# jafarinia/snuffy

Measured on AMD Instinct MI355X. Metric: slides/sec, higher is better.
Workload: dtype f32; 1 GPU; cfgB: MILNet eval forward, 1 bag/step/rank, N=32768 patches D=768 h=6 Lambda=200 (K=200) depth=1 relu mlp x4; parallelism=bag-parallel x1, bags_resident_per_rank=8, launch=hip graph replay, rccl_ranks=0

## Files before the change

### snuffy_amd/csrc/gemm.hip

```cpp
#include <stdlib.h>

#include "mfma.h"
#include "philox.h"

namespace {

struct GemmParams {
    const unsigned short* a;
    const unsigned short* w;
    const float* bias;
    void* c;
    int64_t lda, ldw, ldc;
    int m, n, k;
    int act;
    int tiles_m, tiles_n;
    unsigned long long* trace;
    const float* resid = nullptr;
    int64_t ldr = 0;
    unsigned int* split_cnt = nullptr;
    float* split_slab = nullptr;
    int split_cap = 0, split_rcap = 0;
    const unsigned short* gate = nullptr;
    int64_t ldg = 0;
    const float* colsum = nullptr;
// ... 402 lines not shown
    while (true) {
        const int next = tile + wgs_per_xcd;
        const bool has_next = next < t_hi;
        const Src nxt = tile_src(has_next ? next : tile);
        const bool full = (tile / P.tiles_n + 1) * BM <= P.m && (tile % P.tiles_n + 1) * BN <= P.n;
        for (int s = 0; s < ns; ++s) {
            if constexpr (EPI == 2)
                if (s == 0) preload_x(tile);
            read_frags(rb);
            if (s == ns - 1) load_bias(tile);
            const bool in_tile = s + AHEAD < ns;
            const int exist = has_next ? AHEAD : (ns - 1 - s < AHEAD ? ns - 1 - s : AHEAD);
            if (in_tile)
                stage(cur, s + AHEAD, sb);
            else if (has_next)
                stage(nxt, s + AHEAD - ns, sb);
            if (exist == AHEAD) {
                if (after_epilogue)
                    wait_vmcnt<(AHEAD - 1) * GL + MI * NST>();
                else
                    wait_vmcnt<(AHEAD - 1) * GL>();
            } else if (AHEAD == 3 && exist == 2) {
                wait_vmcnt<GL>();
            } else {
                wait_vmcnt<0>();
            }
            after_epilogue = false;
            rb = rb == NBUF - 1 ? 0 : rb + 1;
            sb = sb == NBUF - 1 ? 0 : sb + 1;
            barrier();
            if (s == 0)
                mma(std::true_type{});
            else
                mma(std::false_type{});
            barrier();
        }
        bias_landed();
#ifdef SNF_GEMM_NOSTORE
        if (false) {
#else
        if (full) {
#endif
            epilogue(tile, std::true_type{});
            after_epilogue = true;
        } else {
            epilogue(tile, std::false_type{});
            wait_vmcnt<0>();
        }
        if (!has_next) break;
        tile = next;
        cur = nxt;
    }
    if (wid < 4) __builtin_amdgcn_s_barrier();
}

template <int ACT, int OUT, bool SPLIT = false, bool GATE = false, bool DROP = false>
__global__ __launch_bounds__(512, 2) void gemm_hl_kernel(GemmParams P) {
    static_assert(!GATE || (OUT == 3 && ACT == SNF_ACT_NONE && !SPLIT), "gemm_hl: the gated form writes an hl image, no activation, no split");
    static_assert(!DROP || (!GATE && (OUT == 1 || OUT == 3)), "gemm_hl: dropout goes with the fp32 and the hl-image outputs");
    constexpr int NI = 4, BN = 256;
    constexpr int ROWL = 128;
    constexpr int IMG = BM * ROWL;
    constexpr int STEP_BYTES = 2 * IMG;
    constexpr int NC = 4 * NI;
    constexpr bool LINE_STORES = (OUT == 1 || OUT == 3) && ACT != SNF_ACT_GELU && ACT != SNF_ACT_SELU;
    extern __shared__ __attribute__((aligned(16))) unsigned char smem[];

    const int lane = threadIdx.x & 63;
    const int wid = __builtin_amdgcn_readfirstlane(threadIdx.x >> 6);
    const int wr = wid >> 2, wc = wid & 3;
    const int ns_all = P.k / BKS;
    unsigned char* const scr = smem + 2 * STEP_BYTES + wid * 4096;

    const int ntiles = P.tiles_m * P.tiles_n;
    const int xcd = blockIdx.x & 7, wg_in_xcd = blockIdx.x >> 3, wgs_per_xcd = gridDim.x >> 3;
    if constexpr (!SPLIT) {
        if (P.split_cap >= 2 && blockIdx.x == 0) {
            for (int i = threadIdx.x; i < 8 * P.split_rcap; i += 512) P.split_cnt[i] = 0u;
            asm volatile("s_waitcnt vmcnt(0)" ::: "memory");
        }
    }
    int t_lo, t_hi;
    {
        const int q = ntiles >> 3, r = ntiles & 7;
        t_lo = xcd < r ? xcd * (q + 1) : r * (q + 1) + (xcd - r) * q;
        t_hi = t_lo + q + (xcd < r ? 1 : 0);
    }
    int sp_part = 0, sp_parts = 1, sp_slot = 0, sp_tile = -1;
    if (P.split_cap >= 2) {
        const int q_x = t_hi - t_lo, full_rounds = q_x / wgs_per_xcd, r = q_x - full_rounds * wgs_per_xcd;
        int sn = r > 0 ? wgs_per_xcd / r : 0;
        if (sn > P.split_cap) sn = P.split_cap;
        if (sn > ns_all / HL_SPLIT_MIN_STEPS) sn = ns_all / HL_SPLIT_MIN_STEPS;
        if (sn >= 2 && r <= P.split_rcap) {
            if constexpr (SPLIT) {
                if (wg_in_xcd < r * sn) {
                    const int jr = wg_in_xcd % r;
                    sp_tile = t_lo + full_rounds * wgs_per_xcd + jr;
                    sp_part = wg_in_xcd / r, sp_parts = sn, sp_slot = xcd * P.split_rcap + jr;
                }
            } else {
                t_hi = t_lo + full_rounds * wgs_per_xcd;
            }
        }
    }
    int tile = t_lo + wg_in_xcd;
    if constexpr (SPLIT) {
        tile = __builtin_amdgcn_readfirstlane(sp_tile);
        sp_part = __builtin_amdgcn_readfirstlane(sp_part), sp_parts = __builtin_amdgcn_readfirstlane(sp_parts);
        sp_slot = __builtin_amdgcn_readfirstlane(sp_slot);
        if (tile < 0) return;
        t_hi = tile + 1;
        asm volatile("" : "+s"(t_hi));
    } else {
        if (tile >= t_hi) return;
    }
    const int s_begin = SPLIT ? __builtin_amdgcn_readfirstlane(sp_part * ns_all / sp_parts) : 0;
    const int ns = SPLIT ? __builtin_amdgcn_readfirstlane((sp_part + 1) * ns_all / sp_parts) - s_begin : ns_all;
    const unsigned short* const a_base = P.a + (SPLIT ? s_begin * 64 : 0);
    const unsigned short* const w_base = P.w + (SPLIT ? s_begin * 64 : 0);

    struct Src {
        int a[4], w[4];
    };
    auto tile_src_mn = [&](int tm, int tn) __attribute__((always_inline)) -> Src {
        Src s;
        int ln = lane;
        asm volatile("" : "+v"(ln));
        const int c = ln & 7;
#pragma unroll
        for (int j = 0; j < 4; ++j) {
            const int row = (4 * wid + j) * 8 + (ln >> 3);
            int grow = tm * BM + row;
            if (grow > P.m - 1) grow = P.m - 1;
            s.a[j] = grow * (int)P.lda + ((c ^ ((row >> 1) & 7)) << 3);
            int wrow = tn * BN + row;
            if (wrow > P.n - 1) wrow = P.n - 1;
            s.w[j] = wrow * (int)P.ldw + ((c ^ (((row >> 1) & 1) | (((row >> 3) & 3) << 1))) << 3);
        }
        return s;
    };
    auto tile_src = [&](int tl) __attribute__((always_inline)) -> Src {
        const int tm = tl / P.tiles_n;
        return tile_src_mn(tm, tl - tm * P.tiles_n);
    };
    auto stage = [&](const Src& s, int kstep, int buf) __attribute__((always_inline)) {
#ifdef X3_NOSTAGE
        return;
#endif
        unsigned char* base = smem + buf * STEP_BYTES;
#pragma unroll
        for (int j = 0; j < 4; ++j) {
            __builtin_amdgcn_global_load_lds((glb_void*)(a_base + s.a[j] + kstep * 64), (lds_void*)(base + (4 * wid + j) * 1024), 16, 0, 0);
            __builtin_amdgcn_global_load_lds((glb_void*)(w_base + s.w[j] + kstep * 64), (lds_void*)(base + IMG + (4 * wid + j) * 1024), 16, 0, 0);
        }
    };

    const int fi = lane & 15, fg = lane >> 4;
    const int fa = (fi >> 1) & 7, fw = ((fi >> 1) & 1) | ((fi >> 2) << 1);
    const int xoff_h = (128 * wr + fi) * ROWL + ((fg ^ fa) << 4), xoff_l = (128 * wr + fi) * ROWL + (((4 + fg) ^ fa) << 4);
    const int wrow0 = IMG + (64 * wc + 8 * (fi >> 2) + (fi & 3)) * ROWL;
    const int woff_h = wrow0 + ((fg ^ fw) << 4), woff_l = wrow0 + (((4 + fg) ^ fw) << 4);

    f32x4 acc[8][NI];
    bf16x8 xf[8], wh[NI], wl[NI];
    f32x4 bv4[NC / 4];

    auto frag = [&](const unsigned char* p) __attribute__((always_inline)) -> bf16x8 {
#ifdef X3_NOREAD
        u32x4 z = {1u, 2u, 3u, (unsigned)lane};
        asm volatile("" : "+v"(z));
        return __builtin_bit_cast(bf16x8, z);
#endif
        return __builtin_bit_cast(bf16x8, *reinterpret_cast<const u32x4*>(p));
    };
#ifdef X3_NOMFMA
#define X3_MFMA(a, b, c) ([&]() { f32x4 t_ = (c); asm volatile("" : "+v"(t_) : "v"(a), "v"(b)); return t_; }())
#else
#define X3_MFMA(a, b, c) __builtin_amdgcn_mfma_f32_16x16x32_bf16(a, b, c, 0, 0, 0)
#endif
    auto load_bias = [&](int tl) __attribute__((always_inline)) {
#pragma unroll
        for (int c4 = 0; c4 < NC / 4; ++c4) bv4[c4] = f32x4{0.f, 0.f, 0.f, 0.f};
        if (P.bias) {
            const int tn = tl % P.tiles_n;
            const int n0 = tn * BN + 64 * wc + 8 * fg;
            const float* bp0 = P.bias + (n0 + 8 <= P.n ? n0 : 0);
            const float* bp1 = P.bias + (n0 + 40 <= P.n ? n0 + 32 : 0);
            asm volatile("global_load_dwordx4 %0, %1, off" : "=v"(bv4[0]) : "v"(bp0) : "memory");
            asm volatile("global_load_dwordx4 %0, %1, off offset:16" : "=v"(bv4[1]) : "v"(bp0) : "memory");
            asm volatile("global_load_dwordx4 %0, %1, off" : "=v"(bv4[2]) : "v"(bp1) : "memory");
            asm volatile("global_load_dwordx4 %0, %1, off offset:16" : "=v"(bv4[3]) : "v"(bp1) : "memory");
        }
    };
    auto bias_landed = [&]() __attribute__((always_inline)) {
#pragma unroll
        for (int c4 = 0; c4 < NC / 4; ++c4) asm volatile("" : "+v"(bv4[c4]));
    };
    auto epilogue = [&](int tl, auto full_t) __attribute__((always_inline)) {
        constexpr bool FULL = decltype(full_t)::value;
        const int tm = tl / P.tiles_n, tn = tl - tm * P.tiles_n;
        const int n0 = tn * BN + 64 * wc + 8 * fg;
        const int row0 = tm * BM + 128 * wr + fi;
        int lane_o = lane;
        asm volatile("" : "+v"(lane_o));
        const int fio = lane_o & 15, fgo = lane_o >> 4;
#pragma unroll
        for (int mi = 0; mi < 8; ++mi) {
            const int row = row0 + 16 * mi;
#pragma unroll
            for (int h = 0; h < NI / 2; ++h) {
                float v[8];
#pragma unroll
                for (int e = 0; e < 8; ++e) v[e] = activate<ACT>(acc[mi][2 * h + (e >> 2)][e & 3] + bv4[2 * h + (e >> 2)][e & 3]);
                const int col = n0 + 32 * h;
                if constexpr (DROP) {
                    const snf::philox_f4 m0 = snf::dropout_mask4(P.drop, 0, P.m, row, P.n, col);
                    const snf::philox_f4 m1 = snf::dropout_mask4(P.drop, 0, P.m, row, P.n, col + 4);
#pragma unroll
                    for (int e = 0; e < 4; ++e) {
                        v[e] *= m0[e];
                        v[4 + e] *= m1[e];
                    }
#pragma unroll
                    for (int e = 0; e < 8; ++e) asm volatile("" : "+v"(v[e]));
                }
#ifdef X3_NOSTORE
                const bool ok = v[0] == 123.456f;
#else
                const bool ok = FULL || (row < P.m && col + 8 <= P.n);
#endif
                if constexpr (GATE) {
                    u32x4 gv = {0u, 0u, 0u, 0u};
                    if (ok) gv = *reinterpret_cast<const u32x4*>(P.gate + (int64_t)row * P.ldg + 64 * (col >> 5) + (col & 31));
#pragma unroll
                    for (int e = 0; e < 4; ++e) {
                        if (!(__uint_as_float(gv[e] << 16) > 0.f)) v[2 * e] = 0.f;
                        if (!(__uint_as_float(gv[e] & 0xffff0000u) > 0.f)) v[2 * e + 1] = 0.f;
                    }
                }
                if constexpr (OUT == 1) {
                    float* dst = reinterpret_cast<float*>(P.c) + (int64_t)row * P.ldc + col;
                    if (P.resid && ok) {
                        const float* rp = P.resid + (int64_t)row * P.ldr + col;
                        const f32x4 r0 = *reinterpret_cast<const f32x4*>(rp), r1 = *reinterpret_cast<const f32x4*>(rp + 4);
#pragma unroll
                        for (int e = 0; e < 4; ++e) {
                            v[e] += r0[e];
                            v[4 + e] += r1[e];
                        }
                    }
                    if constexpr (LINE_STORES) {
                        *reinterpret_cast<f32x4*>(scr + fio * 256 + (((8 * h + 2 * fgo) ^ fio) << 4)) = f32x4{v[0], v[1], v[2], v[3]};
                        *reinterpret_cast<f32x4*>(scr + fio * 256 + (((8 * h + 2 * fgo + 1) ^ fio) << 4)) = f32x4{v[4], v[5], v[6], v[7]};
                    } else if (ok) {
                        *reinterpret_cast<f32x4*>(dst) = f32x4{v[0], v[1], v[2], v[3]};
                        *reinterpret_cast<f32x4*>(dst + 4) = f32x4{v[4], v[5], v[6], v[7]};
                    }
                } else {
                    const u32x4 pk = {cvt_pk_bf16(v[0], v[1]), cvt_pk_bf16(v[2], v[3]), cvt_pk_bf16(v[4], v[5]), cvt_pk_bf16(v[6], v[7])};
                    if constexpr (OUT == 0) {
                        unsigned short* dst = reinterpret_cast<unsigned short*>(P.c) + (int64_t)row * P.ldc + col;
                        if (ok) *reinterpret_cast<u32x4*>(dst) = pk;
                    } else {
                        float lo[8];
#pragma unroll
                        for (int e = 0; e < 8; ++e)
                            lo[e] = v[e] - __uint_as_float((e & 1) ? (pk[e >> 1] & 0xffff0000u) : (pk[e >> 1] << 16));
                        const u32x4 pl = {cvt_pk_bf16(lo[0], lo[1]), cvt_pk_bf16(lo[2], lo[3]), cvt_pk_bf16(lo[4], lo[5]), cvt_pk_bf16(lo[6], lo[7])};
                        unsigned short* dst = reinterpret_cast<unsigned short*>(P.c) + (int64_t)row * P.ldc + 64 * (col >> 5) + (col & 31);
                        if constexpr (LINE_STORES) {
                            *reinterpret_cast<u32x4*>(scr + fio * 256 + (((8 * h + fgo) ^ fio) << 4)) = pk;
                            *reinterpret_cast<u32x4*>(scr + fio * 256 + (((8 * h + 4 + fgo) ^ fio) << 4)) = pl;
                        } else if (ok) {
                            *reinterpret_cast<u32x4*>(dst) = pk;
                            *reinterpret_cast<u32x4*>(dst + 32) = pl;
                        }
                    }
                }
            }
            if constexpr (LINE_STORES) {
                const int lr = lane_o >> 4, lc = lane_o & 15;
                unsigned char* const crow = reinterpret_cast<unsigned char*>(P.c) +
                                            (OUT == 1 ? 4 * (int64_t)(tn * BN + 64 * wc) : 2 * 2 * (int64_t)(tn * BN + 64 * wc));
                const int64_t pitch = (OUT == 1 ? 4 : 2) * P.ldc;
#pragma unroll
                for (int jj = 0; jj < 4; ++jj) {
                    const int r = lr + 4 * jj;
                    const u32x4 val = *reinterpret_cast<const u32x4*>(scr + r * 256 + ((lc ^ r) << 4));
                    const int orow = tm * BM + 128 * wr + 16 * mi + r;
                    const int ocol = tn * BN + 64 * wc + (OUT == 1 ? 4 * lc : 32 * (lc >> 3) + 8 * (lc & 3));
#ifdef X3_NOSTORE
                    const bool ok2 = val[0] == 0x12345678u && orow < 0;
#else
                    const bool ok2 = FULL || (orow < P.m && ocol + (OUT == 1 ? 4 : 8) <= P.n);
#endif
                    if (ok2) *reinterpret_cast<u32x4*>(crow + orow * pitch + 16 * lc) = val;
                }
            }
        }
    };

    Src cur = tile_src(tile);
    stage(cur, 0, 0);
    int buf = 0;
    bool after_epilogue = false;
    while (true) {
        const int next = tile + wgs_per_xcd;
        const bool has_next = next < t_hi;
        const bool full = (tile / P.tiles_n + 1) * BM <= P.m && (tile % P.tiles_n + 1) * BN <= P.n;
        for (int s = 0; s < ns; ++s) {
            if (!(s == 0 && after_epilogue)) wait_vmcnt<0>();
            after_epilogue = false;
            __builtin_amdgcn_sched_barrier(0);
            __builtin_amdgcn_s_barrier();
            __builtin_amdgcn_sched_barrier(0);
            const unsigned char* base = smem + buf * STEP_BYTES;
#pragma unroll
            for (int ni = 0; ni < NI; ++ni) wh[ni] = frag(base + woff_h + (4 * (ni & 1) + 32 * (ni >> 1)) * ROWL);
#pragma unroll
            for (int mi = 0; mi < 8; ++mi) xf[mi] = frag(base + xoff_h + mi * 16 * ROWL);
#pragma unroll
            for (int ni = 0; ni < NI; ++ni) wl[ni] = frag(base + woff_l + (4 * (ni & 1) + 32 * (ni >> 1)) * ROWL);
            __builtin_amdgcn_sched_barrier(0);
            if (s + 1 < ns) {
                stage(cur, s + 1, buf ^ 1);
            } else if (has_next) {
                cur = tile_src(next);
                stage(cur, 0, buf ^ 1);
            }
            __builtin_amdgcn_sched_barrier(0);
            __builtin_amdgcn_s_setprio(1);
            if (s == 0) {
#pragma unroll
                for (int mi = 0; mi < 8; ++mi)
#pragma unroll
                    for (int ni = 0; ni < NI; ++ni) acc[mi][ni] = X3_MFMA(wh[ni], xf[mi], (f32x4{0.f, 0.f, 0.f, 0.f}));
            } else {
#pragma unroll
                for (int mi = 0; mi < 8; ++mi)
#pragma unroll
                    for (int ni = 0; ni < NI; ++ni) acc[mi][ni] = X3_MFMA(wh[ni], xf[mi], acc[mi][ni]);
            }
#pragma unroll
            for (int mi = 0; mi < 8; ++mi) {
#pragma unroll
                for (int ni = 0; ni < NI; ++ni) acc[mi][ni] = X3_MFMA(wl[ni], xf[mi], acc[mi][ni]);
                __builtin_amdgcn_sched_barrier(0);
                xf[mi] = frag(base + xoff_l + mi * 16 * ROWL);
                __builtin_amdgcn_sched_barrier(0);
            }
#pragma unroll
            for (int mi = 0; mi < 8; ++mi)
#pragma unroll
                for (int ni = 0; ni < NI; ++ni) acc[mi][ni] = X3_MFMA(wh[ni], xf[mi], acc[mi][ni]);
            __builtin_amdgcn_s_setprio(0);
            buf ^= 1;
        }
        if constexpr (SPLIT) {
            volatile unsigned int& s_ticket = *reinterpret_cast<volatile unsigned int*>(smem);
            float* slab0 = P.split_slab + (size_t)sp_slot * P.split_cap * (size_t)(BM * BN);
            unsigned tix = threadIdx.x;
            asm volatile("" : "+v"(tix));
            f32x4* mine = reinterpret_cast<f32x4*>(slab0 + (size_t)sp_part * (BM * BN)) + tix;
            wait_vmcnt<0>();
#pragma unroll
            for (int mi = 0; mi < 8; ++mi)
#pragma unroll
                for (int ni = 0; ni < NI; ++ni) mine[(mi * NI + ni) * 512] = acc[mi][ni];
            wait_vmcnt<0>();
            __syncthreads();
            if (tix == 0) {
                __builtin_amdgcn_fence(__ATOMIC_RELEASE, "agent");
                asm volatile("s_waitcnt vmcnt(0)" ::: "memory");
                s_ticket = __hip_atomic_fetch_add(P.split_cnt + sp_slot, 1u, __ATOMIC_RELAXED, __HIP_MEMORY_SCOPE_AGENT);
            }
            __syncthreads();
            if (s_ticket != (unsigned)(sp_parts - 1)) return;
            __syncthreads();
            if (tix == 0) {
                __builtin_amdgcn_fence(__ATOMIC_ACQUIRE, "agent");
                __hip_atomic_store(P.split_cnt + sp_slot, 0u, __ATOMIC_RELAXED, __HIP_MEMORY_SCOPE_AGENT);
            }
            __syncthreads();
#pragma unroll
            for (int mi = 0; mi < 8; ++mi)
#pragma unroll
                for (int ni = 0; ni < NI; ++ni) {
                    f32x4 sum = {0.f, 0.f, 0.f, 0.f};
                    for (int pp = 0; pp < sp_parts; ++pp) {
                        f32x4 v = acc[mi][ni];
                        if (pp != sp_part) v = reinterpret_cast<const f32x4*>(slab0 + (size_t)pp * (BM * BN))[(mi * NI + ni) * 512 + tix];
                        sum = pp == 0 ? v : sum + v;
                    }
                    acc[mi][ni] = sum;
                }
        }
        load_bias(tile);
        wait_vmcnt<0>();
        bias_landed();
        if (full)
            epilogue(tile, std::true_type{});
        else
            epilogue(tile, std::false_type{});
        after_epilogue = true;
        if (!has_next) break;
        tile = next;
    }
}

template <int ACT, int OUT, bool DROP = false>
int launch_hl(const GemmParams& P, hipStream_t s) {
    constexpr int lds = 2 * 2 * BM * 128 + (((OUT == 1 || OUT == 3) && ACT != SNF_ACT_GELU && ACT != SNF_ACT_SELU) ? 8 * 4096 : 0);
    auto kern = [] {
        if constexpr (DROP) return gemm_hl_kernel<ACT, OUT, false, false, true>;
        else return gemm_hl_kernel<ACT, OUT>;
    }();
    static thread_local unsigned long long attr_set_mask = 0;
    if (int rc = snf::lds_opt_in(reinterpret_cast<const void*>(kern), lds, &attr_set_mask, "gemm_hl")) return rc;
    const int ntiles = P.tiles_m * P.tiles_n;
    int grid = snf::cu_count() & ~7;
    if (grid < 8) grid = 8;
    {
        static const int dbg_grid = getenv("SNF_GEMM_HL_GRID") ? atoi(getenv("SNF_GEMM_HL_GRID")) & ~7 : 0;
        if (dbg_grid >= 8 && dbg_grid < grid && P.split_cap < 2) grid = dbg_grid;
    }
    const int per_xcd = (ntiles + 7) / 8;
    if (per_xcd * 8 < grid) grid = per_xcd * 8;
    hipLaunchKernelGGL(kern, dim3(grid), dim3(512), lds, s, P);
    int rc = snf::check_launch("gemm_hl_kernel");
    if (rc || P.split_cap < 2) return rc;
    auto kern2 = [] {
        if constexpr (DROP) return gemm_hl_kernel<ACT, OUT, true, false, true>;
        else return gemm_hl_kernel<ACT, OUT, true>;
    }();
    static thread_local unsigned long long attr_set2_mask = 0;
    if (int rc = snf::lds_opt_in(reinterpret_cast<const void*>(kern2), lds, &attr_set2_mask, "gemm_hl")) return rc;
    hipLaunchKernelGGL(kern2, dim3(grid), dim3(512), lds, s, P);
    return snf::check_launch("gemm_hl_kernel<split>");
}

int launch_hl_gated(const GemmParams& P, hipStream_t s) {
    constexpr int lds = 2 * 2 * BM * 128 + 8 * 4096;
    auto kern = gemm_hl_kernel<SNF_ACT_NONE, 3, false, true>;
    static thread_local unsigned long long attr_set_mask = 0;
    if (int rc = snf::lds_opt_in(reinterpret_cast<const void*>(kern), lds, &attr_set_mask, "gemm_hl")) return rc;
    const int ntiles = P.tiles_m * P.tiles_n;
    int grid = snf::cu_count() & ~7;
    if (grid < 8) grid = 8;
    const int per_xcd = (ntiles + 7) / 8;
    if (per_xcd * 8 < grid) grid = per_xcd * 8;
    hipLaunchKernelGGL(kern, dim3(grid), dim3(512), lds, s, P);
    return snf::check_launch("gemm_hl_kernel<gated>");
}

template <int OUT>
int launch_hl_act(const GemmParams& P, hipStream_t s) {
    switch (P.act) {
        case SNF_ACT_RELU: return launch_hl<SNF_ACT_RELU, OUT>(P, s);
        case SNF_ACT_GELU: return launch_hl<SNF_ACT_GELU, OUT>(P, s);
        case SNF_ACT_LEAKYRELU: return launch_hl<SNF_ACT_LEAKYRELU, OUT>(P, s);
        case SNF_ACT_SELU: return launch_hl<SNF_ACT_SELU, OUT>(P, s);
        default: return launch_hl<SNF_ACT_NONE, OUT>(P, s);
    }
}

template <int NI, int ACT, int OUT, int EPI = 0, int MI = 8, bool DROP = false>
int launch(const GemmParams& P, hipStream_t s) {
    constexpr int lds = NBUF * (A_BYTES + (MI == 8 ? 64 : 32) * NI * ROWB) +
                        ((EPI == 2 || (OUT == 0 && NI == 4 && ACT != SNF_ACT_GELU && ACT != SNF_ACT_SELU)) ? 8 * 4096 : 0);
    auto kern = [] {
        if constexpr (DROP) return gemm_bf16_kernel<NI, ACT, OUT, EPI, MI, true>;
        else return gemm_bf16_kernel<NI, ACT, OUT, EPI, MI>;
    }();
    static thread_local unsigned long long attr_set_mask = 0;
    if (int rc = snf::lds_opt_in(reinterpret_cast<const void*>(kern), lds, &attr_set_mask, "gemm_bf16")) return rc;
    const int ntiles = P.tiles_m * P.tiles_n;
    int grid = snf::cu_count() & ~7;
    if (grid < 8) grid = 8;
    const int per_xcd = (ntiles + 7) / 8;
    if (per_xcd * 8 < grid) grid = per_xcd * 8;
    hipLaunchKernelGGL(kern, dim3(grid), dim3(512), lds, s, P);
    return snf::check_launch("gemm_bf16_kernel");
}

#ifndef SNF_GEMM_128_MI4
#define SNF_GEMM_128_MI4 1
#endif
template <int NI, int ACT, int OUT, int EPI = 0, bool DROP = false>
int launch_tile(const GemmParams& P, hipStream_t s) {
    if constexpr (NI == 2 && SNF_GEMM_128_MI4)
        return launch<4, ACT, OUT, EPI, 4, DROP>(P, s);
    else
        return launch<NI, ACT, OUT, EPI, 8, DROP>(P, s);
}

template <int NI, int OUT>
int launch_act(const GemmParams& P, hipStream_t s) {
    switch (P.act) {
        case SNF_ACT_RELU: return launch_tile<NI, SNF_ACT_RELU, OUT>(P, s);
        case SNF_ACT_GELU: return launch_tile<NI, SNF_ACT_GELU, OUT>(P, s);
        case SNF_ACT_LEAKYRELU: return launch_tile<NI, SNF_ACT_LEAKYRELU, OUT>(P, s);
        case SNF_ACT_SELU: return launch_tile<NI, SNF_ACT_SELU, OUT>(P, s);
        default: return launch_tile<NI, SNF_ACT_NONE, OUT>(P, s);
    }
}

struct SkinnyFrag {
    int dk, chunk_size;
    int64_t chunk_stride;
    float c_exp;
    const int64_t* idx = nullptr;
    int64_t n_rows = 0;
    float* xs = nullptr;
    int64_t ldxs = 0;
    int32_t* map = nullptr;
    const float* resid = nullptr;
    float* out2 = nullptr;
    int64_t ldr = 0, ldo2 = 0;
};
template <bool OUT_BF16, bool FRAG = false>
__global__ __launch_bounds__(512) void skinny_linear_x3_kernel(const float* __restrict__ x, int64_t ldx, const float* __restrict__ w,
                                                                int64_t ldw, const float* __restrict__ bias, int r, int c, int k,
                                                                void* __restrict__ out, int64_t ldo, SkinnyFrag fr = SkinnyFrag{}) {
    constexpr int NW = 8, BATCH = 6;
    __shared__ float red[NW - 1][32 * 32];
    if constexpr (FRAG) {
        const int nrb = (r + 31) >> 5;
        if ((int)blockIdx.y >= nrb) {
            int* sel = reinterpret_cast<int*>(&red[0][0]);
            for (int q = threadIdx.x; q < r; q += 512) sel[q] = (int)fr.idx[q];
            __syncthreads();
            const int64_t i = ((int64_t)(blockIdx.y - nrb) * gridDim.x + blockIdx.x) * 512 + threadIdx.x;
            if (i >= fr.n_rows) return;
            int slot = -1;
            const int me = (int)i;
            for (int q = 0; q < r; ++q) slot = (sel[q] == me) ? q : slot;
            fr.map[i] = slot;
            return;
        }
    }
    const int lane = threadIdx.x & 63, wv = threadIdx.x >> 6;
    const int j = lane & 31, hf = lane >> 5;
    const int row0 = blockIdx.y * 32, col0 = blockIdx.x * 32;
    int xr = row0 + j, wr = col0 + j;
    if (xr > r - 1) xr = r - 1;
    if (wr > c - 1) wr = c - 1;
    const int xr_out = xr;
    bool xs_out = false;
    if constexpr (FRAG) {
        if (fr.idx) {
            int64_t src = fr.idx[xr];
            src = src < 0 ? 0 : (src > fr.n_rows - 1 ? fr.n_rows - 1 : src);
            xr = (int)src;
            xs_out = fr.xs != nullptr && blockIdx.x == 0 && row0 + j < r;
        }
    }
    const int steps = k >> 4, per = (steps + NW - 1) / NW;
    const int s_lo = wv * per, s_hi = s_lo + per < steps ? s_lo + per : steps;
    const float* xp = x + (int64_t)xr * ldx + 8 * hf;
    const float* wp = w + (int64_t)wr * ldw + 8 * hf;
    f32x16 acc;
#pragma unroll
    for (int i = 0; i < 16; ++i) acc[i] = 0.f;
    for (int s0 = s_lo; s0 < s_hi; s0 += BATCH) {
        f32x8 xv[BATCH], wvv[BATCH];
#pragma unroll
        for (int u = 0; u < BATCH; ++u) {
            const int st = s0 + u < s_hi ? s0 + u : s_hi - 1;
            xv[u] = load8(xp + 16 * st);
            wvv[u] = load8(wp + 16 * st);
        }
        __builtin_amdgcn_sched_barrier(0);
        if constexpr (FRAG) {
            if (xs_out) {
#pragma unroll
                for (int u = 0; u < BATCH; ++u)
                    if (s0 + u < s_hi) {
                        float* d8 = fr.xs + (int64_t)xr_out * fr.ldxs + 8 * hf + 16 * (s0 + u);
                        *reinterpret_cast<f32x4*>(d8) = f32x4{xv[u][0], xv[u][1], xv[u][2], xv[u][3]};
                        *reinterpret_cast<f32x4*>(d8 + 4) = f32x4{xv[u][4], xv[u][5], xv[u][6], xv[u][7]};
                    }
            }
        }
#pragma unroll
        for (int u = 0; u < BATCH; ++u) {
            bf16x8 xh, xl, wh, wl;
            const float live = s0 + u < s_hi ? 1.f : 0.f;
            split8(xv[u] * live, xh, xl);
            split8(wvv[u], wh, wl);
            acc = __builtin_amdgcn_mfma_f32_32x32x16_bf16(wl, xh, acc, 0, 0, 0);
            acc = __builtin_amdgcn_mfma_f32_32x32x16_bf16(wh, xl, acc, 0, 0, 0);
            acc = __builtin_amdgcn_mfma_f32_32x32x16_bf16(wh, xh, acc, 0, 0, 0);
        }
    }
    if (wv > 0) {
#pragma unroll
        for (int i = 0; i < 16; ++i) red[wv - 1][i * 64 + lane] = acc[i];
    }
    __syncthreads();
    __shared__ float blk[32][33];
    if (wv == 0) {
#pragma unroll
        for (int i = 0; i < 16; ++i) {
            float v = acc[i];
#pragma unroll
            for (int q = 0; q < NW - 1; ++q) v += red[q][i * 64 + lane];
            const int cl = (i & 3) + 8 * (i >> 2) + 4 * hf;
            blk[j][cl] = v;
        }
    }
    const int bcol = col0 + (threadIdx.x & 31);
    const float bv = (bias && bcol < c) ? bias[bcol] : 0.f;
    __syncthreads();
    if constexpr (FRAG) {
        if (threadIdx.x < 128) {
            const int gq = threadIdx.x >> 5;
            const int ch = row0 / fr.chunk_size, b = (row0 - ch * fr.chunk_size) >> 5;
            int kc = r - ch * fr.chunk_size;
            if (kc > fr.chunk_size) kc = fr.chunk_size;
            const int nkb = fr.chunk_size < r ? (fr.chunk_size + 31) >> 5 : (kc + 31) >> 5, nks = fr.dk >> 4;
            const int a = col0 / fr.dk, cin = col0 - a * fr.dk + 8 * gq;
            const int kb = cin >> 4, hf2 = (cin >> 3) & 1;
            f32x8 v;
#pragma unroll
            for (int e = 0; e < 8; ++e) v[e] = (blk[j][8 * gq + e] + (bias ? bias[col0 + 8 * gq + e] : 0.f)) * fr.c_exp;
            bf16x8 hi, lo;
            split8(v, hi, lo);
            u32x4 uh = __builtin_bit_cast(u32x4, hi), ul = __builtin_bit_cast(u32x4, lo);
            if (row0 + j >= r) uh = ul = u32x4{0u, 0u, 0u, 0u};
            u32x4* dst = reinterpret_cast<u32x4*>(out) + ch * fr.chunk_stride + ((int64_t)(a * nkb + b) * nks * 2 + 2 * kb) * 64 + 32 * hf2 + j;
            dst[0] = uh;
            dst[64] = ul;
        }
        return;
    }
    for (int e = threadIdx.x; e < 32 * 32; e += 512) {
        const int rl = e >> 5, cl = e & 31;
        const int row = row0 + rl, col = col0 + cl;
        if (row < r && col < c) {
            const float v = blk[rl][cl] + bv;
            if constexpr (OUT_BF16) {
                reinterpret_cast<unsigned short*>(out)[(int64_t)row * ldo + col] = (unsigned short)(cvt_pk_bf16(v, 0.f) & 0xffffu);
            } else {
                reinterpret_cast<float*>(out)[(int64_t)row * ldo + col] = v;
                if (fr.out2) fr.out2[(int64_t)row * fr.ldo2 + col] = v + fr.resid[(int64_t)row * fr.ldr + col];
            }
        }
    }
}

}

int snf::skinny_linear_x3_kpfrag(const float* x, int64_t ldx, const float* w, int64_t ldw, const float* bias, int r, int c, int k, int dk,
                                 int chunk_size, int64_t chunk_stride, float c_exp, void* frag, hipStream_t s, const int64_t* idx,
                                 int64_t n_rows, float* xs, int64_t ldxs, int32_t* map) {
    dim3 grid((unsigned)((c + 31) / 32), (unsigned)((r + 31) / 32));
    SkinnyFrag fr;
    fr.dk = dk, fr.chunk_size = chunk_size, fr.chunk_stride = chunk_stride, fr.c_exp = c_exp;
    fr.idx = idx, fr.n_rows = n_rows, fr.xs = xs, fr.ldxs = ldxs, fr.map = idx ? map : nullptr;
// ... 332 lines not shown
```

Measured before the change: 898.4 slides/s.

## Prefetch next-step LDS fragments during MFMA phase with two-ahead global staging

Restructures the GEMM main loop so two stages are issued up front and the barrier, wait and next global stage happen mid-step. Fragments for the next step's W-high and X-high are read from LDS while the current step's final MFMA phase runs. Steps are unrolled in pairs that swap the wh/wl register roles, so reuse needs no extra registers. The aim is to hide LDS read latency and the barrier stall behind MFMA work, at the cost of more complex sync and possible hazards at tile boundaries and in epilogue handling.

```diff
diff --git a/snuffy_amd/csrc/gemm.hip b/snuffy_amd/csrc/gemm.hip
--- a/snuffy_amd/csrc/gemm.hip
+++ b/snuffy_amd/csrc/gemm.hip
@@ -728,60 +728,105 @@
     };
 
     Src cur = tile_src(tile);
-    stage(cur, 0, 0);
+    int st_tile = tile, st_step = 0;
+    auto stage_next = [&](int b) __attribute__((always_inline)) {
+        if (st_tile >= t_hi) return;
+        stage(cur, st_step, b);
+        if (++st_step == ns) {
+            st_step = 0;
+            st_tile += wgs_per_xcd;
+            if (st_tile < t_hi) cur = tile_src(st_tile);
+        }
+    };
+    stage_next(0);
+    const bool second_staged = st_tile < t_hi;
+    stage_next(1);
+    if (second_staged)
+        wait_vmcnt<8>();
+    else
+        wait_vmcnt<0>();
+    __builtin_amdgcn_sched_barrier(0);
+    __builtin_amdgcn_s_barrier();
+    __builtin_amdgcn_sched_barrier(0);
     int buf = 0;
     bool after_epilogue = false;
+
+    auto step = [&](const int s, auto even_t, bf16x8(&WH)[NI], bf16x8(&WL)[NI]) __attribute__((always_inline)) {
+        constexpr bool EVEN = decltype(even_t)::value;
+        const unsigned char* base = smem + buf * STEP_BYTES;
+        const unsigned char* nbase = smem + (buf ^ 1) * STEP_BYTES;
+        if constexpr (EVEN) {
+            if (s == 0) {
+#pragma unroll
+                for (int ni = 0; ni < NI; ++ni) WH[ni] = frag(base + woff_h + (4 * (ni & 1) + 32 * (ni >> 1)) * ROWL);
+#pragma unroll
+                for (int mi = 0; mi < 8; ++mi) xf[mi] = frag(base + xoff_h + mi * 16 * ROWL);
+            }
+        }
+        __builtin_amdgcn_sched_barrier(0);
+        __builtin_amdgcn_s_setprio(1);
+        auto read_wl = [&]() __attribute__((always_inline)) {
+            __builtin_amdgcn_sched_barrier(0);
+#pragma unroll
+            for (int ni = 0; ni < NI; ++ni) WL[ni] = frag(base + woff_l + (4 * (ni & 1) + 32 * (ni >> 1)) * ROWL);
+            __builtin_amdgcn_sched_barrier(0);
+        };
+        if (EVEN && s == 0) {
+#pragma unroll
+            for (int mi = 0; mi < 8; ++mi) {
+#pragma unroll
+                for (int ni = 0; ni < NI; ++ni) acc[mi][ni] = X3_MFMA(WH[ni], xf[mi], (f32x4{0.f, 0.f, 0.f, 0.f}));
+                if (mi == 0) read_wl();
+            }
+        } else {
+#pragma unroll
+            for (int mi = 0; mi < 8; ++mi) {
+#pragma unroll
+                for (int ni = 0; ni < NI; ++ni) acc[mi][ni] = X3_MFMA(WH[ni], xf[mi], acc[mi][ni]);
+                if (mi == 0) read_wl();
+            }
+        }
+#pragma unroll
+        for (int mi = 0; mi < 8; ++mi) {
+#pragma unroll
+            for (int ni = 0; ni < NI; ++ni) acc[mi][ni] = X3_MFMA(WL[ni], xf[mi], acc[mi][ni]);
+            __builtin_amdgcn_sched_barrier(0);
+            xf[mi] = frag(base + xoff_l + mi * 16 * ROWL);
+            __builtin_amdgcn_sched_barrier(0);
+        }
+#pragma unroll
+        for (int mi = 0; mi < 8; ++mi) {
+#pragma unroll
+            for (int ni = 0; ni < NI; ++ni) acc[mi][ni] = X3_MFMA(WH[ni], xf[mi], acc[mi][ni]);
+            __builtin_amdgcn_sched_barrier(0);
+            if (mi == 0) {
+                __builtin_amdgcn_s_setprio(0);
+                asm volatile("s_waitcnt lgkmcnt(0)" ::: "memory");
+                if (!after_epilogue) wait_vmcnt<0>();
+                after_epilogue = false;
+                __builtin_amdgcn_sched_barrier(0);
+                __builtin_amdgcn_s_barrier();
+                __builtin_amdgcn_sched_barrier(0);
+                stage_next(buf);
+                __builtin_amdgcn_sched_barrier(0);
+                __builtin_amdgcn_s_setprio(1);
+#pragma unroll
+                for (int ni = 0; ni < NI; ++ni) WL[ni] = frag(nbase + woff_h + (4 * (ni & 1) + 32 * (ni >> 1)) * ROWL);
+            }
+            xf[mi] = frag(nbase + xoff_h + mi * 16 * ROWL);
+            __builtin_amdgcn_sched_barrier(0);
+        }
+        __builtin_amdgcn_s_setprio(0);
+        buf ^= 1;
+    };
+
     while (true) {
         const int next = tile + wgs_per_xcd;
         const bool has_next = next < t_hi;
         const bool full = (tile / P.tiles_n + 1) * BM <= P.m && (tile % P.tiles_n + 1) * BN <= P.n;
-        for (int s = 0; s < ns; ++s) {
-            if (!(s == 0 && after_epilogue)) wait_vmcnt<0>();
-            after_epilogue = false;
-            __builtin_amdgcn_sched_barrier(0);
-            __builtin_amdgcn_s_barrier();
-            __builtin_amdgcn_sched_barrier(0);
-            const unsigned char* base = smem + buf * STEP_BYTES;
-#pragma unroll
-            for (int ni = 0; ni < NI; ++ni) wh[ni] = frag(base + woff_h + (4 * (ni & 1) + 32 * (ni >> 1)) * ROWL);
-#pragma unroll
-            for (int mi = 0; mi < 8; ++mi) xf[mi] = frag(base + xoff_h + mi * 16 * ROWL);
-#pragma unroll
-            for (int ni = 0; ni < NI; ++ni) wl[ni] = frag(base + woff_l + (4 * (ni & 1) + 32 * (ni >> 1)) * ROWL);
-            __builtin_amdgcn_sched_barrier(0);
-            if (s + 1 < ns) {
-                stage(cur, s + 1, buf ^ 1);
-            } else if (has_next) {
-                cur = tile_src(next);
-                stage(cur, 0, buf ^ 1);
-            }
-            __builtin_amdgcn_sched_barrier(0);
-            __builtin_amdgcn_s_setprio(1);
-            if (s == 0) {
-#pragma unroll
-                for (int mi = 0; mi < 8; ++mi)
-#pragma unroll
-                    for (int ni = 0; ni < NI; ++ni) acc[mi][ni] = X3_MFMA(wh[ni], xf[mi], (f32x4{0.f, 0.f, 0.f, 0.f}));
-            } else {
-#pragma unroll
-                for (int mi = 0; mi < 8; ++mi)
-#pragma unroll
-                    for (int ni = 0; ni < NI; ++ni) acc[mi][ni] = X3_MFMA(wh[ni], xf[mi], acc[mi][ni]);
-            }
-#pragma unroll
-            for (int mi = 0; mi < 8; ++mi) {
-#pragma unroll
-                for (int ni = 0; ni < NI; ++ni) acc[mi][ni] = X3_MFMA(wl[ni], xf[mi], acc[mi][ni]);
-                __builtin_amdgcn_sched_barrier(0);
-                xf[mi] = frag(base + xoff_l + mi * 16 * ROWL);
-                __builtin_amdgcn_sched_barrier(0);
-            }
-#pragma unroll
-            for (int mi = 0; mi < 8; ++mi)
-#pragma unroll
-                for (int ni = 0; ni < NI; ++ni) acc[mi][ni] = X3_MFMA(wh[ni], xf[mi], acc[mi][ni]);
-            __builtin_amdgcn_s_setprio(0);
-            buf ^= 1;
+        for (int s = 0; s < ns; s += 2) {
+            step(s, std::true_type{}, wh, wl);
+            if (s + 1 < ns) step(s + 1, std::false_type{}, wl, wh);
         }
         if constexpr (SPLIT) {
             volatile unsigned int& s_ticket = *reinterpret_cast<volatile unsigned int*>(smem);
```

New measurement: 907.3 slides/s (median of 6 runs). Within noise of the previous version (+1.0%).
